# zju-pi/diff-sampler

Measured on AMD Instinct MI355X. Metric: images/sec (whole node) at NFE=10, EDM CIFAR-10, higher is better.
Workload: dtype fp32; 1 GPU; EDM CIFAR-10 32x32 SongUNet (55.7M params), DPM-Solver++(2M) logSNR NFE=10, batch 256/GPU; launch=eager

## Files before the change

### diff_sampler_amd/csrc/conv3x3_wino.hip

```cpp
#include <type_traits>

#include "igemm_common.h"

namespace igemm {
namespace {

typedef float f32x2 __attribute__((ext_vector_type(2)));

constexpr int WV_NO_NORM = 2, WV_NO_HALO = 4, WV_NO_DMA = 8, WV_NO_EPI = 16;
constexpr int WINO_K = 8;
constexpr int WINO_POS = 2 * 64 * 4;
constexpr int WINO_IMG = 16 * WINO_POS;
constexpr int WINO_NSH = 4;
constexpr int WINO_EPI_LD = 36;

#define DS_WINO_WAIT_VM0() do { __builtin_amdgcn_s_waitcnt(0x0F70); asm volatile("" ::: "memory"); } while (0)
#define DS_WINO_WAIT_VM(n) do { __builtin_amdgcn_s_waitcnt(0x0F70 | (n)); asm volatile("" ::: "memory"); } while (0)

#define DS_WINO_I(n) std::integral_constant<int, (n)>{}
#define DS_WINO_EACH4(F) F(0) F(1) F(2) F(3)
#define DS_WINO_EACH8(F) F(0) F(1) F(2) F(3) F(4) F(5) F(6) F(7)
#define DS_WINO_EACH12(F) F(0) F(1) F(2) F(3) F(4) F(5) F(6) F(7) F(8) F(9) F(10) F(11)
#define DS_WINO_EACH16(F, b) F((b) + 0) F((b) + 1) F((b) + 2) F((b) + 3) F((b) + 4) F((b) + 5) F((b) + 6) F((b) + 7)                \
                             F((b) + 8) F((b) + 9) F((b) + 10) F((b) + 11) F((b) + 12) F((b) + 13) F((b) + 14) F((b) + 15)

template <int NT, int NSH, int NSL, int NORM>
struct WinoHalo {
    struct Regs {
        f32x4 h[NSH];
        f32x4 mu = {0.f, 0.f, 0.f, 0.f}, ga = {1.f, 1.f, 1.f, 1.f}, be = {0.f, 0.f, 0.f, 0.f};
    };
    const int c0, Ctot;
    const int buf;
    unsigned off0[NSH], off1[NSH];
    int lds[NSH];
    const float *a0i, *a1i;
    const float* cpi;
    unsigned c_lane;
    float t[4 * NSH], u[4 * NSH];
    const float* h_src = nullptr;
    unsigned h_sel = 0;

    __device__ __forceinline__ WinoHalo(const KParams& p, float* Hs, int tid, int img0, int r0)
        : c0(p.c0), Ctot(p.c0 + p.c1), buf(p.NP * WINO_K + 4) {
        const int kh_h = tid & 1, WPH = p.WP >> 1;
#pragma unroll
        for (int j = 0; j < NSH; ++j) {
            const int hp = (tid + j * NT) >> 1;
            const int hr = hp / p.WP, hc = hp - hr * p.WP;
            const int y = r0 + hr - 1, x = hc - 1;
            const bool in = hp < p.NP;
            const bool ok = in && (unsigned)y < (unsigned)p.H && (unsigned)x < (unsigned)p.W;
            const int pix = min(max(y, 0), p.H - 1) * p.W + min(max(x, 0), p.W - 1);
            off0[j] = (unsigned)(pix * p.lda0 + kh_h * 4) * 4u;
            off1[j] = (unsigned)(pix * p.lda1 + kh_h * 4) * 4u;
            const int cell = (((kh_h * 2 + (hc & 1)) * p.HP + hr) * WPH + (hc >> 1)) * 4;
            lds[j] = ok ? cell : p.NP * WINO_K;
            if (in && !ok) {
                const f32x4 z = {0.f, 0.f, 0.f, 0.f};
                *reinterpret_cast<f32x4*>(Hs + cell) = z;
                *reinterpret_cast<f32x4*>(Hs + buf + cell) = z;
            }
        }
        a0i = p.a0 + (size_t)img0 * p.HW * p.lda0;
        a1i = p.a1 + (size_t)img0 * p.HW * p.lda1;
        cpi = p.norm + (size_t)img0 * 3 * Ctot;
        c_lane = (unsigned)(kh_h * 16);
    }
    __device__ __forceinline__ void src(int s) {
        const int c = s * WINO_K;
        const bool first = c < c0;
        h_src = first ? a0i + c : a1i + (c - c0);
        h_sel = (unsigned)__builtin_amdgcn_readfirstlane(first ? -1 : 0);
        asm volatile("" : "+s"(h_sel));
    }
    template <int J>
    __device__ __forceinline__ void load1(Regs& R, std::integral_constant<int, J>) {
        if constexpr (J < NSL) {
            const unsigned off = (off0[J] & h_sel) | (off1[J] & ~h_sel);
            R.h[J] = *reinterpret_cast<const f32x4*>(reinterpret_cast<const char*>(h_src) + off);
        }
    }
    template <int I>
    __device__ __forceinline__ void coef1(Regs& R, int s, std::integral_constant<int, I>) {
        if constexpr (NORM != 0) {
            const char* cs = reinterpret_cast<const char*>(cpi + (size_t)I * Ctot + s * WINO_K);
            asm volatile("" : "+v"(c_lane));
            const f32x4 v = *reinterpret_cast<const f32x4*>(cs + c_lane);
            if constexpr (I == 0) R.mu = v; else if constexpr (I == 1) R.ga = v; else R.be = v;
        }
    }
    __device__ __forceinline__ void loads(Regs& R, int s) {
#define DS_WINO_F(j) load1(R, DS_WINO_I(j));
        DS_WINO_EACH4(DS_WINO_F)
#undef DS_WINO_F
        coef1(R, s, DS_WINO_I(0)); coef1(R, s, DS_WINO_I(1)); coef1(R, s, DS_WINO_I(2));
    }
    template <int C, int ST>
    __device__ __forceinline__ void chain(Regs& R, float* hs) {
        constexpr int j = C >> 2, e = C & 3;
        if constexpr (j < NSL) {
            if constexpr (ST == 0 && NORM != 0) {
                t[C] = __builtin_fmaf(R.h[j][e] - R.mu[e], R.ga[e], R.be[e]);
                if constexpr (NORM == 2) u[C] = __expf(-t[C]);
            }
            if constexpr (ST == 1 && NORM == 2) u[C] = __builtin_amdgcn_rcpf(1.0f + u[C]);
            if constexpr (ST == 2) {
                float v = R.h[j][e];
                if constexpr (NORM == 1) v = t[C];
                if constexpr (NORM == 2) v = t[C] * u[C];
                R.h[j][e] = v;
                if constexpr (e == 3) *reinterpret_cast<f32x4*>(hs + lds[j]) = R.h[j];
            }
        }
    }
    __device__ __forceinline__ void store(Regs& R, float* hs) {
#define DS_WINO_F(c) chain<c, 0>(R, hs); chain<c, 1>(R, hs); chain<c, 2>(R, hs);
        DS_WINO_EACH16(DS_WINO_F, 0)
#undef DS_WINO_F
    }
};

template <int NT, int ROWS>
struct WinoSkip {
    static constexpr int STEP = NT / 8, NE = 4 * ROWS / STEP;
    int lds[NE];
    int a_off[4];
    unsigned t0, t1;
    const float* src = nullptr;
    unsigned off = 0;
    int step = 0;

    __device__ __forceinline__ WinoSkip(const KParams& p, int tid, int lane, int row0) {
        const int e_chunk = tid & 7, Wt = p.W >> 1;
#pragma unroll
        for (int j = 0; j < NE; ++j) {
            const int lp = (tid >> 3) + STEP * j;
            const int yl = lp / p.W, x = lp - yl * p.W;
            const int ph = (yl & 1) * 2 + (x & 1), t = (yl >> 1) * Wt + (x >> 1);
            lds[j] = (((ph * 4 + (e_chunk >> 1)) * 2 + (e_chunk & 1)) * ROWS + (t ^ e_chunk)) * 4;
        }
#pragma unroll
        for (int g = 0; g < 4; ++g) a_off[g] = ((lane >> 5) * ROWS + ((row0 + (lane & 31)) ^ (2 * g + (lane >> 5)))) * 4;
        t0 = (unsigned)((tid >> 3) * p.elda0 + e_chunk * 4);
        t1 = (unsigned)((tid >> 3) * p.elda1 + e_chunk * 4);
    }
    __device__ __forceinline__ void sel(const KParams& p, int es, int m0) {
        const int c = es * 32;
        const bool first = c < p.ec0;
        const int ld = first ? p.elda0 : p.elda1;
        src = (first ? p.e0 + c : p.e1 + (c - p.ec0)) + (size_t)m0 * ld;
        step = STEP * ld;
        off = first ? t0 : t1;
    }
    template <int J>
    __device__ __forceinline__ void load1(f32x4* dst, std::integral_constant<int, J>) {
        dst[J] = *reinterpret_cast<const f32x4*>(src + (size_t)(J * step) + off);
    }
};

template <auto KERNEL, int NT, int LDS_MAX>
int wino_launch(KParams& p, int smem, hipStream_t stream) {
    DS_ENSURE_DYN_LDS(KERNEL, LDS_MAX);
    hipLaunchKernelGGL(KERNEL, dim3(grid_1d(p.mtiles, p.ntiles)), dim3(NT), smem, stream, p);
    DS_CHECK_LAUNCH();
    return DS_OK;
}

template <typename F>
int wino_by_norm(const KParams& p, F launch) {
    if (!p.norm) return launch(DS_WINO_I(0));
    return p.norm_act == DS_ACT_SILU ? launch(DS_WINO_I(2)) : launch(DS_WINO_I(1));
}

template <int VAR, int NORM, int NSL>
__global__ void __launch_bounds__(256, 1) conv3x3_wino_kernel(const KParams p) {
    extern __shared__ __attribute__((aligned(16))) float smem[];
    float* Us = smem;
    float* Vs = smem + 2 * WINO_IMG;
    float* Hs = smem + 4 * WINO_IMG;

    const int tid = threadIdx.x, lane = tid & 63;
    const int wave = __builtin_amdgcn_readfirstlane(tid >> 6);
    const int wr = wave >> 1, wc = wave & 1;
    int mt, nt;
    if (!decode_tile(blockIdx.x, p.mtiles, p.ntiles, mt, nt)) return;
    const int m0 = mt * 256, n0 = nt * 64;
    const int img0 = m0 / p.HW;
    const int r0 = (m0 - img0 * p.HW) / p.W;
    const int WPH = p.WP >> 1, Wt = p.W >> 1;
    const int Ctot = p.c0 + p.c1;
    const int nslabs = Ctot / WINO_K;
    constexpr bool kDma = !(VAR & WV_NO_DMA), kHalo = !(VAR & WV_NO_HALO);

    constexpr int kNorm = (VAR & WV_NO_NORM) ? 0 : NORM;
    const int kh_h = tid & 1;
    const int h_buf = p.NP * WINO_K + 4;
    unsigned h_off0[WINO_NSH], h_off1[WINO_NSH];
    int h_lds[WINO_NSH];
#pragma unroll
    for (int j = 0; j < WINO_NSH; ++j) {
        const int hp = (tid + j * 256) >> 1;
        const int hr = hp / p.WP, hc = hp - hr * p.WP;
        const int y = r0 + hr - 1, x = hc - 1;
        const bool in = hp < p.NP;
        const bool ok = in && (unsigned)y < (unsigned)p.H && (unsigned)x < (unsigned)p.W;
        const int pix = min(max(y, 0), p.H - 1) * p.W + min(max(x, 0), p.W - 1);
        h_off0[j] = (unsigned)(pix * p.lda0 + kh_h * 4) * 4u;
        h_off1[j] = (unsigned)(pix * p.lda1 + kh_h * 4) * 4u;
        const int cell = (((kh_h * 2 + (hc & 1)) * p.HP + hr) * WPH + (hc >> 1)) * 4;
        h_lds[j] = ok ? cell : p.NP * WINO_K;
        if (in && !ok) {
            const f32x4 z = {0.f, 0.f, 0.f, 0.f};
            *reinterpret_cast<f32x4*>(Hs + cell) = z;
            *reinterpret_cast<f32x4*>(Hs + h_buf + cell) = z;
        }
    }
    const float* a0i = p.a0 + (size_t)img0 * p.HW * p.lda0;
    const float* a1i = p.a1 + (size_t)img0 * p.HW * p.lda1;
    const float* cpi = p.norm + (size_t)img0 * 3 * Ctot;
    unsigned c_lane = (unsigned)(kh_h * 16);
    struct HaloRegs {
        f32x4 h[WINO_NSH];
        f32x4 mu = {0.f, 0.f, 0.f, 0.f}, ga = {1.f, 1.f, 1.f, 1.f}, be = {0.f, 0.f, 0.f, 0.f};
    };
    HaloRegs hreg;
    float h_t[4 * WINO_NSH], h_u[4 * WINO_NSH];
    const float* h_src = nullptr;
    unsigned h_sel = 0;
    auto halo_src = [&](int s) {
        const int c = s * WINO_K;
        const bool first = c < p.c0;
        h_src = first ? a0i + c : a1i + (c - p.c0);
        h_sel = (unsigned)__builtin_amdgcn_readfirstlane(first ? -1 : 0);
        asm volatile("" : "+s"(h_sel));
    };
    auto halo_load1 = [&](HaloRegs& R, auto J) {
        constexpr int j = decltype(J)::value;
        if constexpr (j >= NSL) return;
        const unsigned off = (h_off0[j] & h_sel) | (h_off1[j] & ~h_sel);
        R.h[j] = *reinterpret_cast<const f32x4*>(reinterpret_cast<const char*>(h_src) + off);
    };
    auto coef_load1 = [&](HaloRegs& R, int s, auto I) {
        constexpr int i = decltype(I)::value;
        if constexpr (NORM != 0) {
            const char* cs = reinterpret_cast<const char*>(cpi + (size_t)i * Ctot + s * WINO_K);
            asm volatile("" : "+v"(c_lane));
            const f32x4 v = *reinterpret_cast<const f32x4*>(cs + c_lane);
            if constexpr (i == 0) R.mu = v; else if constexpr (i == 1) R.ga = v; else R.be = v;
        }
    };
    auto halo_chain = [&](HaloRegs& R, float* hs, auto C, auto ST) {
        constexpr int c = decltype(C)::value, st = decltype(ST)::value, j = c >> 2, e = c & 3;
        if constexpr (j >= NSL) return;
        if constexpr (st == 0 && kNorm != 0) {
            h_t[c] = __builtin_fmaf(R.h[j][e] - R.mu[e], R.ga[e], R.be[e]);
            if constexpr (kNorm == 2) h_u[c] = __expf(-h_t[c]);
        }
        if constexpr (st == 1 && kNorm == 2) h_u[c] = __builtin_amdgcn_rcpf(1.0f + h_u[c]);
        if constexpr (st == 2) {
            float v = R.h[j][e];
            if constexpr (kNorm == 1) v = h_t[c];
            if constexpr (kNorm == 2) v = h_t[c] * h_u[c];
            R.h[j][e] = v;
            if constexpr (e == 3) *reinterpret_cast<f32x4*>(hs + h_lds[j]) = R.h[j];
        }
    };

    const int t_t = (tid >> 1) & 63, cpl = tid & 1, kh_t = tid >> 7;
    const int t_ty = t_t / Wt, t_tx = t_t - t_ty * Wt;
    const int h_rd = ((kh_t * 2 * p.HP + 2 * t_ty) * WPH + t_tx) * 4 + cpl * 2;
    const int h_par = p.HP * WPH * 4;
    const int v_wr = (kh_t * 64 + t_t) * 4 + cpl * 2;
    f32x2 t_d[4][4], t_r[4];
    auto tr_read1 = [&](const float* hs, auto I) {
        constexpr int i = decltype(I)::value >> 2, j = decltype(I)::value & 3;
        t_d[i][j] = *reinterpret_cast<const f32x2*>(hs + h_rd + (j & 1) * h_par + i * WPH * 4 + (j >> 1) * 4);
    };
    auto tr_write1 = [&](float* vs, auto I) {
        constexpr int i = decltype(I)::value >> 2, j = decltype(I)::value & 3;
        if constexpr (j == 0) {
#pragma unroll
            for (int q = 0; q < 4; ++q)
                t_r[q] = i == 0 ? t_d[0][q] - t_d[2][q] : i == 1 ? t_d[1][q] + t_d[2][q] : i == 2 ? t_d[2][q] - t_d[1][q] : t_d[1][q] - t_d[3][q];
        }
        const f32x2 v = j == 0 ? t_r[0] - t_r[2] : j == 1 ? t_r[1] + t_r[2] : j == 2 ? t_r[2] - t_r[1] : t_r[1] - t_r[3];
        *reinterpret_cast<f32x2*>(vs + v_wr + (i * 4 + j) * WINO_POS) = v;
    };

    const float* u_src = p.b + (size_t)nt * nslabs * WINO_IMG;
    unsigned u_lane = (unsigned)tid * 16u;
    auto u_dma1 = [&](const float* src, float* ubuf, auto I) {
        constexpr int i = decltype(I)::value;
        float* dst = ubuf + (i * 256 + wave * 64) * 4;
        typedef const __attribute__((address_space(1))) void* gptr_t;
        typedef __attribute__((address_space(3))) void* lptr_t;
        const char* us = reinterpret_cast<const char*>(src + i * 1024);
        asm volatile("" : "+s"(us));
        asm volatile("" : "+v"(u_lane));
        __builtin_amdgcn_global_load_lds((gptr_t)(us + u_lane), (lptr_t)(dst), 16, 0, 0);
    };

    f32x16 acc[16];
#pragma unroll
    for (int q = 0; q < 16; ++q)
#pragma unroll
        for (int r = 0; r < 16; ++r) acc[q][r] = 0.f;
    const int a_off = ((lane >> 5) * 64 + wr * 32 + (lane & 31)) * 4;
    const int b_off = ((lane >> 5) * 64 + wc * 32 + (lane & 31)) * 4;

#define DS_WINO_LOADS(R, sl)                                                                                                           \
    halo_load1(R, DS_WINO_I(0)); halo_load1(R, DS_WINO_I(1)); halo_load1(R, DS_WINO_I(2)); halo_load1(R, DS_WINO_I(3));                \
    coef_load1(R, sl, DS_WINO_I(0)); coef_load1(R, sl, DS_WINO_I(1)); coef_load1(R, sl, DS_WINO_I(2));

    halo_src(0);
    DS_WINO_LOADS(hreg, 0)
    {
        HaloRegs hreg1;
        const int s1 = min(1, nslabs - 1);
        halo_src(s1);
        DS_WINO_LOADS(hreg1, s1)
        DS_RACE_SKEW(wave);
#define DS_WINO_F(i) u_dma1(u_src, Us, DS_WINO_I(i)); u_dma1(u_src, Us, DS_WINO_I((i) + 4));
        DS_WINO_EACH4(DS_WINO_F)
#undef DS_WINO_F
        DS_RACE_SKEW(wave);
#define DS_WINO_CHAIN1(c) halo_chain(hreg, Hs, DS_WINO_I(c), DS_WINO_I(0)); halo_chain(hreg, Hs, DS_WINO_I(c), DS_WINO_I(1));          \
                          halo_chain(hreg, Hs, DS_WINO_I(c), DS_WINO_I(2));
        DS_WINO_EACH16(DS_WINO_CHAIN1, 0)
#undef DS_WINO_CHAIN1
        DS_RACE_SKEW(wave);
#define DS_WINO_CHAIN1(c) halo_chain(hreg1, Hs + h_buf, DS_WINO_I(c), DS_WINO_I(0)); halo_chain(hreg1, Hs + h_buf, DS_WINO_I(c), DS_WINO_I(1)); \
                          halo_chain(hreg1, Hs + h_buf, DS_WINO_I(c), DS_WINO_I(2));
        DS_WINO_EACH16(DS_WINO_CHAIN1, 0)
#undef DS_WINO_CHAIN1
    }
    {
        const int s2 = min(2, nslabs - 1);
        halo_src(s2);
        DS_WINO_LOADS(hreg, s2)
    }
    __syncthreads();
#define DS_WINO_F(i) tr_read1(Hs, DS_WINO_I(i));
    DS_WINO_EACH16(DS_WINO_F, 0)
#undef DS_WINO_F
    DS_RACE_SKEW(wave);
#define DS_WINO_F(i) tr_write1(Vs, DS_WINO_I(i));
    DS_WINO_EACH16(DS_WINO_F, 0)
#undef DS_WINO_F
    DS_WINO_WAIT_VM0();
    __syncthreads();

    f32x4 fa[2][4], fb[2][4];
    int s = 0;
    do {
        const int par = s & 1;
        const float* ub = Us + par * WINO_IMG;
        const float* vb = Vs + par * WINO_IMG;
        float* ubn = Us + (par ^ 1) * WINO_IMG;
        float* vbn = Vs + (par ^ 1) * WINO_IMG;
        float* hb = Hs + par * h_buf;
        const float* hbn = Hs + (par ^ 1) * h_buf;
        const int s1 = min(s + 1, nslabs - 1), s3 = min(s + 3, nslabs - 1);
        const float* un = u_src + (size_t)s1 * WINO_IMG;
// ... 221 lines not shown
    const int wave = __builtin_amdgcn_readfirstlane(tid >> 6);
    int mt, nt;
    if (!decode_tile(blockIdx.x, p.mtiles, p.ntiles, mt, nt)) return;
    const int m0 = mt * 128, n0 = nt * 128;
    const int img0 = m0 / p.HW;
    const int r0 = (m0 - img0 * p.HW) / p.W;
    const int WPH = p.WP >> 1, Wt = p.W >> 1;
    const int Ctot = p.c0 + p.c1;
    const int nslabs = Ctot / WINO_K;

    using Halo = WinoHalo<256, WN_NSH, NSL, NORM>;
    Halo halo(p, Hs, tid, img0, r0);
    const int h_buf = halo.buf;
    typename Halo::Regs hreg;
    auto halo_load1 = [&](typename Halo::Regs& R, auto J) { halo.load1(R, J); };
    auto coef_load1 = [&](typename Halo::Regs& R, int sl, auto I) { halo.coef1(R, sl, I); };

    const int t_t = (tid >> 1) & 31, cpl = tid & 1, kh_t = wave & 1, half = wave >> 1;
    const int t_ty = t_t / Wt, t_tx = t_t - t_ty * Wt;
    const int h_rd = ((kh_t * 2 * p.HP + 2 * t_ty + half) * WPH + t_tx) * 4 + cpl * 2;
    const int h_par = p.HP * WPH * 4;
    const int v_wr = (kh_t * 32 + t_t) * 4 + cpl * 2 + half * 8 * WN_POS;
    f32x2 t_e[3][4];
    auto tr_read1 = [&](const float* hs, auto I) {
        constexpr int i = decltype(I)::value >> 2, j = decltype(I)::value & 3;
        t_e[i][j] = *reinterpret_cast<const f32x2*>(hs + h_rd + (j & 1) * h_par + i * WPH * 4 + (j >> 1) * 4);
    };
    auto tr_write = [&](float* vs) {
        f32x2 ra[4], rb[4];
        if (half == 0) {
#pragma unroll
            for (int q = 0; q < 4; ++q) { ra[q] = t_e[0][q] - t_e[2][q]; rb[q] = t_e[1][q] + t_e[2][q]; }
        } else {
#pragma unroll
            for (int q = 0; q < 4; ++q) { ra[q] = t_e[1][q] - t_e[0][q]; rb[q] = t_e[0][q] - t_e[2][q]; }
        }
#pragma unroll
        for (int i = 0; i < 2; ++i) {
            const f32x2* t_r = i == 0 ? ra : rb;
#pragma unroll
            for (int j = 0; j < 4; ++j) {
                const f32x2 v = j == 0 ? t_r[0] - t_r[2] : j == 1 ? t_r[1] + t_r[2] : j == 2 ? t_r[2] - t_r[1] : t_r[1] - t_r[3];
                *reinterpret_cast<f32x2*>(vs + v_wr + (i * 4 + j) * WN_POS) = v;
            }
        }
    };

    const float* u_src = p.b + (size_t)(2 * nt + (wave >> 1)) * nslabs * WINO_IMG;
    unsigned b_lane = (unsigned)(((lane >> 5) * 64 + (wave & 1) * 32 + (lane & 31)) * 16);
    f32x4 fa[2][4], fb[2][4];
    typedef const __attribute__((address_space(1))) f32x4* gf4_t;
    auto b_load1 = [&](const float* src, auto G, auto I) {
        constexpr int g = decltype(G)::value, i = decltype(I)::value;
        const char* us = reinterpret_cast<const char*>(src + (g * 4 + i) * WINO_POS);
        asm volatile("" : "+s"(us));
        asm volatile("" : "+v"(b_lane));
        fb[g & 1][i] = *(gf4_t)(us + b_lane);
    };

    f32x16 acc[16];
#pragma unroll
    for (int q = 0; q < 16; ++q)
#pragma unroll
        for (int r = 0; r < 16; ++r) acc[q][r] = 0.f;
    const int a_off = ((lane >> 5) * 32 + (lane & 31)) * 4;

    halo.src(0);
    halo.loads(hreg, 0);
    {
        typename Halo::Regs hreg1;
        const int s1 = min(1, nslabs - 1);
        halo.src(s1);
        halo.loads(hreg1, s1);
#define DS_WINO_F(i) b_load1(u_src, DS_WINO_I(0), DS_WINO_I(i));
        DS_WINO_EACH4(DS_WINO_F)
#undef DS_WINO_F
        DS_RACE_SKEW(wave);
        halo.store(hreg, Hs);
        DS_RACE_SKEW(wave);
        halo.store(hreg1, Hs + h_buf);
    }
    {
        const int s2 = min(2, nslabs - 1);
        halo.src(s2);
        halo.loads(hreg, s2);
    }
    __syncthreads();
#define DS_WINO_TR1(i) tr_read1(Hs, DS_WINO_I(i));
    DS_WINO_EACH12(DS_WINO_TR1)
#undef DS_WINO_TR1
    DS_RACE_SKEW(wave);
    tr_write(Vs);
    DS_WINO_WAIT_VM0();
    __syncthreads();

    int s = 0;
    do {
        const int par = s & 1;
        const float* vb = Vs + par * WN_IMG;
        float* vbn = Vs + (par ^ 1) * WN_IMG;
        float* hb = Hs + par * h_buf;
        const float* hbn = Hs + (par ^ 1) * h_buf;
        const int s1 = min(s + 1, nslabs - 1), s3 = min(s + 3, nslabs - 1);
        const float* uc = u_src + (size_t)s * WINO_IMG;
        const float* un = u_src + (size_t)s1 * WINO_IMG;
        auto a_read = [&](auto G, auto I) {
            constexpr int g = decltype(G)::value, i = decltype(I)::value;
            fa[g & 1][i] = *reinterpret_cast<const f32x4*>(vb + (g * 4 + i) * WN_POS + a_off);
        };
#define DS_WINO_TR1(i) tr_read1(hbn, DS_WINO_I(i));
        DS_WINO_EACH12(DS_WINO_TR1)
#undef DS_WINO_TR1
        DS_RACE_SKEW(wave);
        halo.store(hreg, hb);
        halo.src(s3);
        DS_RACE_SKEW(wave);
        tr_write(vbn);
        auto fill = [&](auto K) {
            constexpr int k = decltype(K)::value, g = k >> 4, q = k & 15;
            if constexpr (q < 4) {
                if constexpr (g < 3) b_load1(uc, DS_WINO_I(g + 1), DS_WINO_I(q));
                else b_load1(un, DS_WINO_I(0), DS_WINO_I(q));
            } else if constexpr (k < 7) {
                halo_load1(hreg, DS_WINO_I(k - 4));
            } else if constexpr (k < 10) {
                coef_load1(hreg, s3, DS_WINO_I(k - 7));
            } else if constexpr (q >= 10 && q < 14 && g < 3) {
                a_read(DS_WINO_I(g + 1), DS_WINO_I(q - 10));
            }
        };
#define DS_WINO_STEP(k)                                                                                                                \
        acc[((k) >> 4) * 4 + ((k) & 3)] = __builtin_amdgcn_mfma_f32_32x32x2f32(fa[((k) >> 4) & 1][(k) & 3][((k) >> 2) & 3],            \
                                                                               fb[((k) >> 4) & 1][(k) & 3][((k) >> 2) & 3],            \
                                                                               acc[((k) >> 4) * 4 + ((k) & 3)], 0, 0, 0);              \
        fill(DS_WINO_I(k));                                                                                                            \
        __builtin_amdgcn_sched_barrier(0);
#define DS_WINO_F(i) a_read(DS_WINO_I(0), DS_WINO_I(i));
        DS_WINO_EACH4(DS_WINO_F)
#undef DS_WINO_F
        __builtin_amdgcn_sched_barrier(0);
        DS_WINO_EACH16(DS_WINO_STEP, 0)
        DS_WINO_EACH16(DS_WINO_STEP, 16)
        DS_WINO_EACH16(DS_WINO_STEP, 32)
        DS_WINO_EACH16(DS_WINO_STEP, 48)
#undef DS_WINO_STEP
        __syncthreads();
    } while (++s < nslabs);

    f32x16 Y[4];
#pragma unroll
    for (int a = 0; a < 2; ++a) {
        f32x16 t[4];
#pragma unroll
        for (int j = 0; j < 4; ++j) t[j] = a == 0 ? acc[j] + acc[4 + j] + acc[8 + j] : acc[4 + j] - acc[8 + j] - acc[12 + j];
        Y[a * 2 + 0] = t[0] + t[1] + t[2];
        Y[a * 2 + 1] = t[1] - t[2] - t[3];
    }

    const int nextra = (p.ec0 + p.ec1) / 32;
    if (nextra > 0) {
        const float* wsk = p.b + (size_t)(p.N / 64) * nslabs * WINO_IMG + (size_t)(2 * nt + (wave >> 1)) * nextra * 2048;
        WinoSkip<256, 32> skip(p, tid, lane, 0);
        auto e_load1 = [&](f32x4* dst, auto J) { skip.load1(dst, J); };
        f32x4 ga[2][4], gb[2];
        auto w_load1 = [&](int es, auto G) {
            constexpr int g = decltype(G)::value;
            const char* ws = reinterpret_cast<const char*>(wsk + (size_t)es * 2048 + g * WINO_POS);
            asm volatile("" : "+s"(ws));
            asm volatile("" : "+v"(b_lane));
            gb[g & 1] = *(gf4_t)(ws + b_lane);
        };

        f32x4 ereg[4];
        {
            f32x4 ereg0[4];
            w_load1(0, DS_WINO_I(0));
            skip.sel(p, 0, m0);
#define DS_WINO_F(j) e_load1(ereg0, DS_WINO_I(j));
            DS_WINO_EACH4(DS_WINO_F)
#undef DS_WINO_F
            skip.sel(p, min(1, nextra - 1), m0);
#define DS_WINO_F(j) e_load1(ereg, DS_WINO_I(j));
            DS_WINO_EACH4(DS_WINO_F)
#undef DS_WINO_F
            DS_RACE_SKEW(wave);
#pragma unroll
            for (int j = 0; j < 4; ++j) *reinterpret_cast<f32x4*>(Vs + skip.lds[j]) = ereg0[j];
        }
        __syncthreads();

        int es = 0;
        do {
            const float* vb = smem + (es & 1) * WN_IMG;
            float* vn = smem + ((es + 1) & 1) * WN_IMG;
            const int es1 = min(es + 1, nextra - 1);
            skip.sel(p, min(es + 2, nextra - 1), m0);
            auto a_read = [&](auto G, auto I) {
                constexpr int g = decltype(G)::value, i = decltype(I)::value;
                ga[g & 1][i] = *reinterpret_cast<const f32x4*>(vb + (i * 4 + g) * WN_POS + skip.a_off[g]);
            };
            auto fill = [&](auto K) {
                constexpr int k = decltype(K)::value, g = k >> 4, q = k & 15;
                if constexpr (q == 0) {
                    if constexpr (g < 3) w_load1(es, DS_WINO_I(g + 1));
                    else w_load1(es1, DS_WINO_I(0));
                } else if constexpr (q < 5) {
                    if constexpr (g < 3) a_read(DS_WINO_I(g + 1), DS_WINO_I(q - 1));
                } else if constexpr (k < 9) {
                    if constexpr (k == 5) DS_RACE_SKEW(wave);
                    *reinterpret_cast<f32x4*>(vn + skip.lds[k - 5]) = ereg[k - 5];
                } else if constexpr (k < 13) {
                    e_load1(ereg, DS_WINO_I(k - 9));
                }
            };
#define DS_WINO_STEP(k)                                                                                                                \
            Y[(k) & 3] = __builtin_amdgcn_mfma_f32_32x32x2f32(ga[((k) >> 4) & 1][(k) & 3][((k) >> 2) & 3], gb[((k) >> 4) & 1][((k) >> 2) & 3], \
                                                              Y[(k) & 3], 0, 0, 0);                                                    \
            fill(DS_WINO_I(k));                                                                                                        \
            __builtin_amdgcn_sched_barrier(0);
#define DS_WINO_F(i) a_read(DS_WINO_I(0), DS_WINO_I(i));
            DS_WINO_EACH4(DS_WINO_F)
#undef DS_WINO_F
            __builtin_amdgcn_sched_barrier(0);
            DS_WINO_EACH16(DS_WINO_STEP, 0)
            DS_WINO_EACH16(DS_WINO_STEP, 16)
            DS_WINO_EACH16(DS_WINO_STEP, 32)
            DS_WINO_EACH16(DS_WINO_STEP, 48)
#undef DS_WINO_STEP
            __syncthreads();
        } while (++es < nextra);
    }

    float* stage = smem + wave * 32 * WINO_EPI_LD;
    const int c4 = (lane & 7) * 4;
    const int col = n0 + wave * 32 + c4;
    f32x4 cb = {0.f, 0.f, 0.f, 0.f}, cvu = {0.f, 0.f, 0.f, 0.f};
    if (p.colbias) cb = *reinterpret_cast<const f32x4*>(p.colbias + col);
    if (p.cbias) cvu = *reinterpret_cast<const f32x4*>(p.cbias + (size_t)(p.cbias_bcast ? 0 : img0) * p.cbias_ld + col);
    const float acc_scale = __builtin_bit_cast(float, __builtin_amdgcn_readfirstlane(__builtin_bit_cast(int, p.acc_scale)));
    const float scale = __builtin_bit_cast(float, __builtin_amdgcn_readfirstlane(__builtin_bit_cast(int, p.scale)));
    int e_row[4];
#pragma unroll
    for (int pass = 0; pass < 4; ++pass) {
        const int tl = pass * 8 + (lane >> 3);
        const int ty = tl / Wt, tx = tl - ty * Wt;
        e_row[pass] = m0 + 2 * ty * p.W + 2 * tx;
    }
#pragma unroll
    for (int a = 0; a < 2; ++a) {
        f32x4 st_s = {0.f, 0.f, 0.f, 0.f}, st_q = {0.f, 0.f, 0.f, 0.f};
#pragma unroll
        for (int b = 0; b < 2; ++b) {
            const f32x16 y = Y[a * 2 + b];
            f32x4 rv[4];
            if (p.res) {
#pragma unroll
                for (int pass = 0; pass < 4; ++pass)
                    rv[pass] = __builtin_nontemporal_load(reinterpret_cast<const f32x4*>(p.res + (size_t)(e_row[pass] + a * p.W + b) * p.res_ld + col));
            }
#pragma unroll
            for (int r = 0; r < 16; ++r) stage[((r & 3) + 8 * (r >> 2) + 4 * (lane >> 5)) * WINO_EPI_LD + (lane & 31)] = y[r];
#pragma unroll
            for (int pass = 0; pass < 4; ++pass) {
                f32x4 v = *reinterpret_cast<const f32x4*>(stage + (pass * 8 + (lane >> 3)) * WINO_EPI_LD + c4);
                v *= acc_scale;
                v += cb;
                if (p.cbias) v += cvu;
                if (p.res) v += rv[pass];
                v *= scale;
                if (p.act == DS_ACT_SILU) {
#pragma unroll
                    for (int q = 0; q < 4; ++q) v[q] = ds_silu(v[q]);
                }
                __builtin_nontemporal_store(v, reinterpret_cast<f32x4*>(p.out + (size_t)(e_row[pass] + a * p.W + b) * p.ldo + col));
                st_s += v; st_q += v * v;
            }
        }
        if (p.stats) {
#pragma unroll
            for (int q = 0; q < 4; ++q) {
                st_s[q] += __shfl_xor(st_s[q], 8); st_s[q] += __shfl_xor(st_s[q], 16); st_s[q] += __shfl_xor(st_s[q], 32);
                st_q[q] += __shfl_xor(st_q[q], 8); st_q[q] += __shfl_xor(st_q[q], 16); st_q[q] += __shfl_xor(st_q[q], 32);
            }
            if (lane < 8) {
                float* sp = p.stats + (size_t)((m0 >> 6) + a) * 2 * p.N + col;
                *reinterpret_cast<f32x4*>(sp) = st_s;
                *reinterpret_cast<f32x4*>(sp + p.N) = st_q;
            }
        }
    }
}

int launch_wino_n128(KParams& p, hipStream_t stream) {
    const int smem = (2 * WN_IMG + 2 * (p.NP * WINO_K + 4)) * (int)sizeof(float);
    return wino_by_norm(p, [&](auto NORM) {
        constexpr int norm = decltype(NORM)::value;
        return p.NP * 2 <= 2 * 256 ? wino_launch<wino_n128_kernel<norm, 2>, 256, 64 * 1024>(p, smem, stream)
                                   : wino_launch<wino_n128_kernel<norm, 3>, 256, 64 * 1024>(p, smem, stream);
    });
}

constexpr int W8_NSH = 1;
constexpr int W8_XCH = 4 * 16 * 64;

template <int NORM>
__global__ void __launch_bounds__(512, 1) wino_w8_kernel(const KParams p) {
    extern __shared__ __attribute__((aligned(16))) float smem[];
    float* Vs = smem;
    float* Hs = smem + 2 * WN_IMG;

    const int tid = threadIdx.x, lane = tid & 63;
    const int wave = __builtin_amdgcn_readfirstlane(tid >> 6);
    const int cg = wave & 3, ph = wave >> 2;
    int mt, nt;
    if (!decode_tile(blockIdx.x, p.mtiles, p.ntiles, mt, nt)) return;
    const int m0 = mt * 128, n0 = nt * 128;
    const int img0 = m0 / p.HW;
    const int r0 = (m0 - img0 * p.HW) / p.W;
    const int WPH = p.WP >> 1, Wt = p.W >> 1;
    const int Ctot = p.c0 + p.c1;
    const int nslabs = Ctot / WINO_K;

    using Halo = WinoHalo<512, W8_NSH, W8_NSH, NORM>;
    Halo halo(p, Hs, tid, img0, r0);
    const int h_buf = halo.buf;
    typename Halo::Regs hreg;
    auto halo_load1 = [&](typename Halo::Regs& R, auto J) { halo.load1(R, J); };
    auto coef_load1 = [&](typename Halo::Regs& R, int sl, auto I) { halo.coef1(R, sl, I); };

    const int t_t = (tid >> 1) & 31, cpl = tid & 1, kh_t = wave & 1, t_row = wave >> 1;
    const int t_ty = t_t / Wt, t_tx = t_t - t_ty * Wt;
    const int h_rd0 = ((kh_t * 2 * p.HP + 2 * t_ty + (t_row == 0 ? 0 : 1)) * WPH + t_tx) * 4 + cpl * 2;
    const int h_rd1 = ((kh_t * 2 * p.HP + 2 * t_ty + (t_row == 3 ? 3 : 2)) * WPH + t_tx) * 4 + cpl * 2;
    const int h_par = p.HP * WPH * 4;
    const int v_wr = (kh_t * 32 + t_t) * 4 + cpl * 2 + t_row * 4 * WN_POS;
    f32x2 t_e[2][4];
    auto tr_read1 = [&](const float* hs, auto I) {
        constexpr int i = decltype(I)::value >> 2, j = decltype(I)::value & 3;
        t_e[i][j] = *reinterpret_cast<const f32x2*>(hs + (i == 0 ? h_rd0 : h_rd1) + (j & 1) * h_par + (j >> 1) * 4);
    };
    auto tr_write = [&](float* vs) {
        f32x2 t_r[4];
        if (t_row == 1) {
#pragma unroll
            for (int q = 0; q < 4; ++q) t_r[q] = t_e[0][q] + t_e[1][q];
        } else if (t_row == 2) {
#pragma unroll
            for (int q = 0; q < 4; ++q) t_r[q] = t_e[1][q] - t_e[0][q];
        } else {
#pragma unroll
            for (int q = 0; q < 4; ++q) t_r[q] = t_e[0][q] - t_e[1][q];
        }
#pragma unroll
        for (int j = 0; j < 4; ++j) {
            const f32x2 v = j == 0 ? t_r[0] - t_r[2] : j == 1 ? t_r[1] + t_r[2] : j == 2 ? t_r[2] - t_r[1] : t_r[1] - t_r[3];
            *reinterpret_cast<f32x2*>(vs + v_wr + j * WN_POS) = v;
        }
    };

    const float* u_src = p.b + (size_t)(2 * nt + (cg >> 1)) * nslabs * WINO_IMG + ph * 8 * WINO_POS;
    unsigned b_lane = (unsigned)(((lane >> 5) * 64 + (cg & 1) * 32 + (lane & 31)) * 16);
    f32x4 fa[2][4], fb[2][4];
    typedef const __attribute__((address_space(1))) f32x4* gf4_t;
    auto b_load1 = [&](const float* src, auto G, auto I) {
        constexpr int g = decltype(G)::value, i = decltype(I)::value;
        const char* us = reinterpret_cast<const char*>(src + (g * 4 + i) * WINO_POS);
        asm volatile("" : "+s"(us));
        asm volatile("" : "+v"(b_lane));
        fb[g & 1][i] = *(gf4_t)(us + b_lane);
    };

    f32x16 acc[8];
#pragma unroll
    for (int q = 0; q < 8; ++q)
#pragma unroll
        for (int r = 0; r < 16; ++r) acc[q][r] = 0.f;
    const int a_off = ((lane >> 5) * 32 + (lane & 31)) * 4 + ph * 8 * WN_POS;

    halo.src(0);
    halo.loads(hreg, 0);
    {
        typename Halo::Regs hreg1;
        const int s1 = min(1, nslabs - 1);
        halo.src(s1);
        halo.loads(hreg1, s1);
#define DS_WINO_F(i) b_load1(u_src, DS_WINO_I(0), DS_WINO_I(i));
        DS_WINO_EACH4(DS_WINO_F)
#undef DS_WINO_F
        DS_RACE_SKEW(wave);
        halo.store(hreg, Hs);
        DS_RACE_SKEW(wave);
        halo.store(hreg1, Hs + h_buf);
    }
    {
        const int s2 = min(2, nslabs - 1);
        halo.src(s2);
        halo.loads(hreg, s2);
    }
    __syncthreads();
#define DS_WINO_TR1(i) tr_read1(Hs, DS_WINO_I(i));
    DS_WINO_EACH8(DS_WINO_TR1)
#undef DS_WINO_TR1
    DS_RACE_SKEW(wave);
    tr_write(Vs);
    DS_WINO_WAIT_VM0();
    __syncthreads();

    int s = 0;
    do {
        const int par = s & 1;
        const float* vb = Vs + par * WN_IMG;
        float* vbn = Vs + (par ^ 1) * WN_IMG;
        float* hb = Hs + par * h_buf;
        const float* hbn = Hs + (par ^ 1) * h_buf;
        const int s1 = min(s + 1, nslabs - 1), s3 = min(s + 3, nslabs - 1);
        const float* uc = u_src + (size_t)s * WINO_IMG;
        const float* un = u_src + (size_t)s1 * WINO_IMG;
        auto a_read = [&](auto G, auto I) {
            constexpr int g = decltype(G)::value, i = decltype(I)::value;
            fa[g & 1][i] = *reinterpret_cast<const f32x4*>(vb + (g * 4 + i) * WN_POS + a_off);
        };
#define DS_WINO_TR1(i) tr_read1(hbn, DS_WINO_I(i));
        DS_WINO_EACH8(DS_WINO_TR1)
#undef DS_WINO_TR1
        DS_RACE_SKEW(wave);
        halo.store(hreg, hb);
        halo.src(s3);
        DS_RACE_SKEW(wave);
        tr_write(vbn);
        auto fill = [&](auto K) {
            constexpr int k = decltype(K)::value, g = k >> 4, q = k & 15;
            if constexpr (q < 4) {
                if constexpr (g == 0) b_load1(uc, DS_WINO_I(1), DS_WINO_I(q));
                else b_load1(un, DS_WINO_I(0), DS_WINO_I(q));
            } else if constexpr (k == 4) {
                halo_load1(hreg, DS_WINO_I(0));
            } else if constexpr (k < 8) {
                coef_load1(hreg, s3, DS_WINO_I(k - 5));
            } else if constexpr (k >= 10 && k < 14) {
                a_read(DS_WINO_I(1), DS_WINO_I(k - 10));
            }
        };
#define DS_WINO_STEP(k)                                                                                                                \
        acc[((k) >> 4) * 4 + ((k) & 3)] = __builtin_amdgcn_mfma_f32_32x32x2f32(fa[((k) >> 4) & 1][(k) & 3][((k) >> 2) & 3],            \
                                                                               fb[((k) >> 4) & 1][(k) & 3][((k) >> 2) & 3],            \
                                                                               acc[((k) >> 4) * 4 + ((k) & 3)], 0, 0, 0);              \
        fill(DS_WINO_I(k));                                                                                                            \
        __builtin_amdgcn_sched_barrier(0);
#define DS_WINO_F(i) a_read(DS_WINO_I(0), DS_WINO_I(i));
        DS_WINO_EACH4(DS_WINO_F)
#undef DS_WINO_F
        __builtin_amdgcn_sched_barrier(0);
        DS_WINO_EACH16(DS_WINO_STEP, 0)
        DS_WINO_EACH16(DS_WINO_STEP, 16)
#undef DS_WINO_STEP
        __syncthreads();
    } while (++s < nslabs);

    f32x16 Y[2];
    {
        float* xw = smem + wave * W8_XCH + lane * 4;
        const float* xr = smem + (wave ^ 4) * W8_XCH + lane * 4;
        DS_RACE_SKEW(wave);
#pragma unroll
        for (int q = 0; q < 4; ++q) {
            const f32x16 m = ph == 0 ? acc[4 + q] : acc[q];
#pragma unroll
            for (int r4 = 0; r4 < 4; ++r4) {
                const f32x4 v = {m[4 * r4], m[4 * r4 + 1], m[4 * r4 + 2], m[4 * r4 + 3]};
                *reinterpret_cast<f32x4*>(xw + (q * 4 + r4) * 256) = v;
            }
        }
        __syncthreads();
        f32x16 t[4];
#pragma unroll
        for (int j = 0; j < 4; ++j) {
            f32x16 o;
#pragma unroll
            for (int r4 = 0; r4 < 4; ++r4) {
                const f32x4 v = *reinterpret_cast<const f32x4*>(xr + (j * 4 + r4) * 256);
                o[4 * r4] = v[0]; o[4 * r4 + 1] = v[1]; o[4 * r4 + 2] = v[2]; o[4 * r4 + 3] = v[3];
            }
            if (ph == 0) t[j] = acc[j] + acc[4 + j] + o;
            else t[j] = o - acc[j] - acc[4 + j];
        }
        Y[0] = t[0] + t[1] + t[2];
        Y[1] = t[1] - t[2] - t[3];
    }

    const int nextra = (p.ec0 + p.ec1) / 32;
    if (nextra > 0) {
        __syncthreads();
        const float* wsk = p.b + (size_t)(p.N / 64) * nslabs * WINO_IMG + (size_t)(2 * nt + (cg >> 1)) * nextra * 2048;
        WinoSkip<512, 32> skip(p, tid, lane, 0);
        auto e_load1 = [&](f32x4* dst, auto J) { skip.load1(dst, J); };
        f32x4 ga[2][2], gb[4];
        auto w_load1 = [&](int es, auto G) {
            constexpr int g = decltype(G)::value;
            const char* ws = reinterpret_cast<const char*>(wsk + (size_t)es * 2048 + g * WINO_POS);
            asm volatile("" : "+s"(ws));
            asm volatile("" : "+v"(b_lane));
            gb[g] = *(gf4_t)(ws + b_lane);
        };

        f32x4 ereg[2];
        {
            f32x4 ereg0[2];
            w_load1(0, DS_WINO_I(0)); w_load1(0, DS_WINO_I(1)); w_load1(0, DS_WINO_I(2)); w_load1(0, DS_WINO_I(3));
            skip.sel(p, 0, m0);
            e_load1(ereg0, DS_WINO_I(0)); e_load1(ereg0, DS_WINO_I(1));
            skip.sel(p, min(1, nextra - 1), m0);
            e_load1(ereg, DS_WINO_I(0)); e_load1(ereg, DS_WINO_I(1));
            DS_RACE_SKEW(wave);
#pragma unroll
            for (int j = 0; j < 2; ++j) *reinterpret_cast<f32x4*>(Vs + skip.lds[j]) = ereg0[j];
        }
        __syncthreads();

        int es = 0;
        do {
            const float* vb = smem + (es & 1) * WN_IMG + ph * 8 * WN_POS;
            float* vn = smem + ((es + 1) & 1) * WN_IMG;
            const int es1 = min(es + 1, nextra - 1);
            skip.sel(p, min(es + 2, nextra - 1), m0);
            auto a_read = [&](auto G, auto I) {
                constexpr int g = decltype(G)::value, i = decltype(I)::value;
                ga[g & 1][i] = *reinterpret_cast<const f32x4*>(vb + (i * 4 + g) * WN_POS + skip.a_off[g]);
            };
            auto fill = [&](auto K) {
                constexpr int k = decltype(K)::value, g = k >> 3, q = k & 7;
                if constexpr (q == 0) {
                    if constexpr (g >= 1) w_load1(es1, DS_WINO_I(g - 1));
                } else if constexpr (q < 3) {
                    if constexpr (g < 3) a_read(DS_WINO_I(g + 1), DS_WINO_I(q - 1));
                } else if constexpr (k < 5) {
                    if constexpr (k == 3) DS_RACE_SKEW(wave);
                    *reinterpret_cast<f32x4*>(vn + skip.lds[k - 3]) = ereg[k - 3];
                } else if constexpr (k < 7) {
                    e_load1(ereg, DS_WINO_I(k - 5));
                } else if constexpr (k == 31) {
                    w_load1(es1, DS_WINO_I(3));
                }
            };
#define DS_WINO_STEP(k)                                                                                                                \
            Y[(k) & 1] = __builtin_amdgcn_mfma_f32_32x32x2f32(ga[((k) >> 3) & 1][(k) & 1][((k) >> 1) & 3], gb[(k) >> 3][((k) >> 1) & 3], \
                                                              Y[(k) & 1], 0, 0, 0);                                                    \
            fill(DS_WINO_I(k));                                                                                                        \
            __builtin_amdgcn_sched_barrier(0);
            a_read(DS_WINO_I(0), DS_WINO_I(0)); a_read(DS_WINO_I(0), DS_WINO_I(1));
            __builtin_amdgcn_sched_barrier(0);
            DS_WINO_EACH16(DS_WINO_STEP, 0)
            DS_WINO_EACH16(DS_WINO_STEP, 16)
#undef DS_WINO_STEP
            __syncthreads();
        } while (++es < nextra);
    }

    float* stage = smem + (wave ^ 4) * W8_XCH;
    const int c4 = (lane & 7) * 4;
    const int col = n0 + cg * 32 + c4;
    f32x4 cb = {0.f, 0.f, 0.f, 0.f}, cvu = {0.f, 0.f, 0.f, 0.f};
    if (p.colbias) cb = *reinterpret_cast<const f32x4*>(p.colbias + col);
    if (p.cbias) cvu = *reinterpret_cast<const f32x4*>(p.cbias + (size_t)(p.cbias_bcast ? 0 : img0) * p.cbias_ld + col);
    const float acc_scale = __builtin_bit_cast(float, __builtin_amdgcn_readfirstlane(__builtin_bit_cast(int, p.acc_scale)));
    const float scale = __builtin_bit_cast(float, __builtin_amdgcn_readfirstlane(__builtin_bit_cast(int, p.scale)));
    int e_row[4];
#pragma unroll
    for (int pass = 0; pass < 4; ++pass) {
        const int tl = pass * 8 + (lane >> 3);
        const int ty = tl / Wt, tx = tl - ty * Wt;
        e_row[pass] = m0 + (2 * ty + ph) * p.W + 2 * tx;
    }
    f32x4 st_s = {0.f, 0.f, 0.f, 0.f}, st_q = {0.f, 0.f, 0.f, 0.f};
#pragma unroll
    for (int b = 0; b < 2; ++b) {
        const f32x16 y = Y[b];
        f32x4 rv[4];
        if (p.res) {
#pragma unroll
            for (int pass = 0; pass < 4; ++pass)
                rv[pass] = __builtin_nontemporal_load(reinterpret_cast<const f32x4*>(p.res + (size_t)(e_row[pass] + b) * p.res_ld + col));
        }
#pragma unroll
        for (int r = 0; r < 16; ++r) stage[((r & 3) + 8 * (r >> 2) + 4 * (lane >> 5)) * WINO_EPI_LD + (lane & 31)] = y[r];
#pragma unroll
        for (int pass = 0; pass < 4; ++pass) {
            f32x4 v = *reinterpret_cast<const f32x4*>(stage + (pass * 8 + (lane >> 3)) * WINO_EPI_LD + c4);
            v *= acc_scale;
            v += cb;
            if (p.cbias) v += cvu;
            if (p.res) v += rv[pass];
            v *= scale;
            if (p.act == DS_ACT_SILU) {
#pragma unroll
                for (int q = 0; q < 4; ++q) v[q] = ds_silu(v[q]);
            }
            __builtin_nontemporal_store(v, reinterpret_cast<f32x4*>(p.out + (size_t)(e_row[pass] + b) * p.ldo + col));
            st_s += v; st_q += v * v;
        }
    }
    if (p.stats) {
#pragma unroll
        for (int q = 0; q < 4; ++q) {
            st_s[q] += __shfl_xor(st_s[q], 8); st_s[q] += __shfl_xor(st_s[q], 16); st_s[q] += __shfl_xor(st_s[q], 32);
            st_q[q] += __shfl_xor(st_q[q], 8); st_q[q] += __shfl_xor(st_q[q], 16); st_q[q] += __shfl_xor(st_q[q], 32);
        }
        if (lane < 8) {
            float* sp = p.stats + (size_t)((m0 >> 6) + ph) * 2 * p.N + col;
            *reinterpret_cast<f32x4*>(sp) = st_s;
            *reinterpret_cast<f32x4*>(sp + p.N) = st_q;
        }
    }
}

int launch_wino_w8(KParams& p, hipStream_t stream) {
    const int kloop = (2 * WN_IMG + 2 * (p.NP * WINO_K + 4)) * (int)sizeof(float), xch = 8 * W8_XCH * (int)sizeof(float);
    return wino_by_norm(p, [&](auto NORM) {
        return wino_launch<wino_w8_kernel<decltype(NORM)::value>, 512, 160 * 1024>(p, kloop > xch ? kloop : xch, stream);
    });
}

template <int VAR>
int launch_wino(KParams& p, hipStream_t stream) {
    const int smem = (4 * WINO_IMG + 2 * (p.NP * WINO_K + 4)) * (int)sizeof(float);
    return wino_by_norm(p, [&](auto NORM) {
        constexpr int norm = decltype(NORM)::value;
        return p.NP * 2 <= 3 * 256 ? wino_launch<conv3x3_wino_kernel<VAR, norm, 3>, 256, 160 * 1024>(p, smem, stream)
                                   : wino_launch<conv3x3_wino_kernel<VAR, norm, 4>, 256, 160 * 1024>(p, smem, stream);
    });
}

#undef DS_WINO_EACH16
#undef DS_WINO_EACH12
#undef DS_WINO_EACH8
#undef DS_WINO_EACH4
#undef DS_WINO_I

}

bool conv3x3_wino_applicable(const KParams& p) {
    if (p.taps != 9 || p.stride != 1 || p.splits != 1 || (p.ec0 & 31) || (p.ec1 & 31)) return false;
    if ((p.H & 1) || (p.W & 1) || p.W < 4 || p.W > 64 || p.HW % 256 || 256 % p.W || ((256 / p.W) & 1)) return false;
    if ((p.N & 63) || (p.c0 % WINO_K) || (p.c1 % WINO_K) || !p.vec_ok || p.out_planar || p.out_f16 || p.res_f16 || p.rowbias) return false;
    if (p.act != DS_ACT_NONE && p.act != DS_ACT_SILU) return false;
    const int np = (256 / p.W + 2) * (p.W + 2);
    if (np * 2 > WINO_NSH * 256 || (4 * WINO_IMG + 2 * (np * WINO_K + 4)) * (int)sizeof(float) > 160 * 1024) return false;
    return p.M % 256 == 0;
}

int launch_conv3x3_wino(KParams& p, hipStream_t stream) {
    if (!conv3x3_wino_applicable(p)) return DS_E_SHAPE;
    p.TH = 256 / p.W; p.nimg = 1; p.HP = p.TH + 2; p.WP = p.W + 2; p.NP = p.HP * p.WP;
    p.mtiles = p.M / 256; p.ntiles = p.N / 64; p.n_begin = 0;
#ifdef DS_CONV_ABLATIONS
    if (p.t_variant & 0x10000) {
        switch (p.t_variant & 31) {
            case 2: return launch_wino<2>(p, stream);
            case 4: return launch_wino<4>(p, stream);
            case 8: return launch_wino<8>(p, stream);
            case 16: return launch_wino<16>(p, stream);
            case 28: return launch_wino<28>(p, stream);
            default: break;
        }
    }
#endif
    if (!(p.t_variant & 1024) && p.N % 128 == 0) {
        p.TH = 128 / p.W; p.HP = p.TH + 2; p.NP = p.HP * p.WP;
        p.mtiles = p.M / 128; p.ntiles = p.N / 128;
        const bool w8 = (p.W == 16 || p.W == 32) && !(p.t_variant & 32768);
        return w8 ? launch_wino_w8(p, stream) : launch_wino_n128(p, stream);
    }
    return launch_wino<0>(p, stream);
}

}
```

Measured before the change: 510.5 images/sec.

## Deepen w8 Winograd pipeline with triple V buffers and four halo buffers

The w8 Winograd conv kernel now keeps three transformed-input (V) LDS buffers and four halo buffers. The prologue preloads four slabs of halo and transforms two ahead. In the main loop, the next slab's A-fragment reads and the halo transform reads are spread across the MFMA steps, so LDS latency hides behind compute instead of sitting at the top of each iteration. This costs more LDS per block and more live registers, which may limit occupancy or cause spills. Ablation switches are added to turn each lookahead off.

```diff
diff --git a/diff_sampler_amd/csrc/conv3x3_wino.hip b/diff_sampler_amd/csrc/conv3x3_wino.hip
--- a/diff_sampler_amd/csrc/conv3x3_wino.hip
+++ b/diff_sampler_amd/csrc/conv3x3_wino.hip
@@ -24,7 +24,7 @@
 #define DS_WINO_EACH16(F, b) F((b) + 0) F((b) + 1) F((b) + 2) F((b) + 3) F((b) + 4) F((b) + 5) F((b) + 6) F((b) + 7)                \
                              F((b) + 8) F((b) + 9) F((b) + 10) F((b) + 11) F((b) + 12) F((b) + 13) F((b) + 14) F((b) + 15)
 
-template <int NT, int NSH, int NSL, int NORM>
+template <int NT, int NSH, int NSL, int NORM, int NB = 2>
 struct WinoHalo {
     struct Regs {
         f32x4 h[NSH];
@@ -60,6 +60,8 @@
                 const f32x4 z = {0.f, 0.f, 0.f, 0.f};
                 *reinterpret_cast<f32x4*>(Hs + cell) = z;
                 *reinterpret_cast<f32x4*>(Hs + buf + cell) = z;
+#pragma unroll
+                for (int b = 2; b < NB; ++b) *reinterpret_cast<f32x4*>(Hs + b * buf + cell) = z;
             }
         }
         a0i = p.a0 + (size_t)img0 * p.HW * p.lda0;
@@ -887,12 +889,26 @@
 
 constexpr int W8_NSH = 1;
 constexpr int W8_XCH = 4 * 16 * 64;
-
+constexpr int W8_VR = 3;
+constexpr int W8_HB = 4;
+
+#ifdef DS_CONV_ABLATIONS
+constexpr int WV_NO_AHEAD_A = 32, WV_NO_AHEAD_T = 64;
+#define DS_W8_KERNEL(norm, var) wino_w8_kernel<norm, var>
+template <int NORM, int VAR = 0>
+#else
+#define DS_W8_KERNEL(norm, var) wino_w8_kernel<norm>
 template <int NORM>
+#endif
 __global__ void __launch_bounds__(512, 1) wino_w8_kernel(const KParams p) {
+#ifdef DS_CONV_ABLATIONS
+    constexpr bool kAheadA = !(VAR & WV_NO_AHEAD_A), kAheadT = !(VAR & WV_NO_AHEAD_T);
+#else
+    constexpr bool kAheadA = true, kAheadT = true;
+#endif
     extern __shared__ __attribute__((aligned(16))) float smem[];
     float* Vs = smem;
-    float* Hs = smem + 2 * WN_IMG;
+    float* Hs = smem + W8_VR * WN_IMG;
 
     const int tid = threadIdx.x, lane = tid & 63;
     const int wave = __builtin_amdgcn_readfirstlane(tid >> 6);
@@ -906,7 +922,7 @@
     const int Ctot = p.c0 + p.c1;
     const int nslabs = Ctot / WINO_K;
 
-    using Halo = WinoHalo<512, W8_NSH, W8_NSH, NORM>;
+    using Halo = WinoHalo<512, W8_NSH, W8_NSH, NORM, W8_HB>;
     Halo halo(p, Hs, tid, img0, r0);
     const int h_buf = halo.buf;
     typename Halo::Regs hreg;
@@ -962,57 +978,76 @@
         for (int r = 0; r < 16; ++r) acc[q][r] = 0.f;
     const int a_off = ((lane >> 5) * 32 + (lane & 31)) * 4 + ph * 8 * WN_POS;
 
-    halo.src(0);
-    halo.loads(hreg, 0);
+    const int last = nslabs - 1;
     {
-        typename Halo::Regs hreg1;
-        const int s1 = min(1, nslabs - 1);
-        halo.src(s1);
-        halo.loads(hreg1, s1);
+        typename Halo::Regs h0, h1, h2, h3;
+        halo.src(0);
+        halo.loads(h0, 0);
+        halo.src(min(1, last));
+        halo.loads(h1, min(1, last));
+        halo.src(min(2, last));
+        halo.loads(h2, min(2, last));
+        halo.src(min(3, last));
+        halo.loads(h3, min(3, last));
 #define DS_WINO_F(i) b_load1(u_src, DS_WINO_I(0), DS_WINO_I(i));
         DS_WINO_EACH4(DS_WINO_F)
 #undef DS_WINO_F
         DS_RACE_SKEW(wave);
-        halo.store(hreg, Hs);
-        DS_RACE_SKEW(wave);
-        halo.store(hreg1, Hs + h_buf);
-    }
-    {
-        const int s2 = min(2, nslabs - 1);
-        halo.src(s2);
-        halo.loads(hreg, s2);
-    }
+        halo.store(h0, Hs + 2 * h_buf);
+        DS_RACE_SKEW(wave);
+        halo.store(h1, Hs + 3 * h_buf);
+        DS_RACE_SKEW(wave);
+        halo.store(h2, Hs);
+        DS_RACE_SKEW(wave);
+        halo.store(h3, Hs + h_buf);
+    }
+    halo.src(min(4, last));
+    halo.loads(hreg, min(4, last));
     __syncthreads();
-#define DS_WINO_TR1(i) tr_read1(Hs, DS_WINO_I(i));
+#define DS_WINO_TR1(i) tr_read1(Hs + 2 * h_buf, DS_WINO_I(i));
     DS_WINO_EACH8(DS_WINO_TR1)
 #undef DS_WINO_TR1
     DS_RACE_SKEW(wave);
     tr_write(Vs);
+#define DS_WINO_TR1(i) tr_read1(Hs + 3 * h_buf, DS_WINO_I(i));
+    DS_WINO_EACH8(DS_WINO_TR1)
+#undef DS_WINO_TR1
+    DS_RACE_SKEW(wave);
+    tr_write(Vs + WN_IMG);
+#define DS_WINO_TR1(i) tr_read1(Hs, DS_WINO_I(i));
+    DS_WINO_EACH8(DS_WINO_TR1)
+#undef DS_WINO_TR1
     DS_WINO_WAIT_VM0();
     __syncthreads();
+#define DS_WINO_F(i) fa[0][i] = *reinterpret_cast<const f32x4*>(Vs + (i) * WN_POS + a_off);
+    DS_WINO_EACH4(DS_WINO_F)
+#undef DS_WINO_F
 
     int s = 0;
+    int v0 = 0, v1 = WN_IMG, v2 = 2 * WN_IMG;
     do {
         const int par = s & 1;
-        const float* vb = Vs + par * WN_IMG;
-        float* vbn = Vs + (par ^ 1) * WN_IMG;
+        const float* vb = Vs + v0;
+        const float* vb1 = Vs + v1;
+        float* vb2 = Vs + v2;
         float* hb = Hs + par * h_buf;
         const float* hbn = Hs + (par ^ 1) * h_buf;
-        const int s1 = min(s + 1, nslabs - 1), s3 = min(s + 3, nslabs - 1);
+        const int s1 = min(s + 1, last), s5 = min(s + 5, last);
         const float* uc = u_src + (size_t)s * WINO_IMG;
         const float* un = u_src + (size_t)s1 * WINO_IMG;
-        auto a_read = [&](auto G, auto I) {
+        auto a_read = [&](const float* v, auto G, auto I) {
             constexpr int g = decltype(G)::value, i = decltype(I)::value;
-            fa[g & 1][i] = *reinterpret_cast<const f32x4*>(vb + (g * 4 + i) * WN_POS + a_off);
+            fa[g & 1][i] = *reinterpret_cast<const f32x4*>(v + (g * 4 + i) * WN_POS + a_off);
         };
-#define DS_WINO_TR1(i) tr_read1(hbn, DS_WINO_I(i));
-        DS_WINO_EACH8(DS_WINO_TR1)
-#undef DS_WINO_TR1
+        if constexpr (!kAheadT) {
+#pragma unroll
+            for (int i = 0; i < 8; ++i) asm volatile("" : "+v"(t_e[i >> 2][i & 3]));
+        }
         DS_RACE_SKEW(wave);
         halo.store(hreg, hb);
-        halo.src(s3);
-        DS_RACE_SKEW(wave);
-        tr_write(vbn);
+        halo.src(s5);
+        DS_RACE_SKEW(wave);
+        tr_write(vb2);
         auto fill = [&](auto K) {
             constexpr int k = decltype(K)::value, g = k >> 4, q = k & 15;
             if constexpr (q < 4) {
@@ -1021,9 +1056,18 @@
             } else if constexpr (k == 4) {
                 halo_load1(hreg, DS_WINO_I(0));
             } else if constexpr (k < 8) {
-                coef_load1(hreg, s3, DS_WINO_I(k - 5));
+                coef_load1(hreg, s5, DS_WINO_I(k - 5));
             } else if constexpr (k >= 10 && k < 14) {
-                a_read(DS_WINO_I(1), DS_WINO_I(k - 10));
+                a_read(vb, DS_WINO_I(1), DS_WINO_I(k - 10));
+            } else if constexpr (k >= 24 && k < 28) {
+                if constexpr (kAheadA) a_read(vb1, DS_WINO_I(0), DS_WINO_I(k - 24));
+            } else if constexpr (!kAheadT) {
+            } else if constexpr (k == 8 || k == 9) {
+                tr_read1(hbn, DS_WINO_I(k - 8));
+            } else if constexpr (k == 14 || k == 15) {
+                tr_read1(hbn, DS_WINO_I(k - 12));
+            } else if constexpr (k >= 20 && k < 24) {
+                tr_read1(hbn, DS_WINO_I(k - 16));
             }
         };
 #define DS_WINO_STEP(k)                                                                                                                \
@@ -1032,14 +1076,13 @@
                                                                                acc[((k) >> 4) * 4 + ((k) & 3)], 0, 0, 0);              \
         fill(DS_WINO_I(k));                                                                                                            \
         __builtin_amdgcn_sched_barrier(0);
-#define DS_WINO_F(i) a_read(DS_WINO_I(0), DS_WINO_I(i));
-        DS_WINO_EACH4(DS_WINO_F)
-#undef DS_WINO_F
         __builtin_amdgcn_sched_barrier(0);
         DS_WINO_EACH16(DS_WINO_STEP, 0)
         DS_WINO_EACH16(DS_WINO_STEP, 16)
 #undef DS_WINO_STEP
         __syncthreads();
+        const int v = v0;
+        v0 = v1; v1 = v2; v2 = v;
     } while (++s < nslabs);
 
     f32x16 Y[2];
@@ -1198,12 +1241,14 @@
     }
 }
 
+template <int VAR = 0>
 int launch_wino_w8(KParams& p, hipStream_t stream) {
-    const int kloop = (2 * WN_IMG + 2 * (p.NP * WINO_K + 4)) * (int)sizeof(float), xch = 8 * W8_XCH * (int)sizeof(float);
+    const int kloop = (W8_VR * WN_IMG + W8_HB * (p.NP * WINO_K + 4)) * (int)sizeof(float), xch = 8 * W8_XCH * (int)sizeof(float);
     return wino_by_norm(p, [&](auto NORM) {
-        return wino_launch<wino_w8_kernel<decltype(NORM)::value>, 512, 160 * 1024>(p, kloop > xch ? kloop : xch, stream);
+        return wino_launch<DS_W8_KERNEL(decltype(NORM)::value, VAR), 512, 160 * 1024>(p, kloop > xch ? kloop : xch, stream);
     });
 }
+#undef DS_W8_KERNEL
 
 template <int VAR>
 int launch_wino(KParams& p, hipStream_t stream) {
@@ -1239,6 +1284,14 @@
     p.mtiles = p.M / 256; p.ntiles = p.N / 64; p.n_begin = 0;
 #ifdef DS_CONV_ABLATIONS
     if (p.t_variant & 0x10000) {
+        const int w8v = p.t_variant & (WV_NO_AHEAD_A | WV_NO_AHEAD_T);
+        if (w8v && p.N % 128 == 0 && (p.W == 16 || p.W == 32)) {
+            p.TH = 128 / p.W; p.HP = p.TH + 2; p.NP = p.HP * p.WP;
+            p.mtiles = p.M / 128; p.ntiles = p.N / 128;
+            return w8v == WV_NO_AHEAD_A   ? launch_wino_w8<WV_NO_AHEAD_A>(p, stream)
+                   : w8v == WV_NO_AHEAD_T ? launch_wino_w8<WV_NO_AHEAD_T>(p, stream)
+                                          : launch_wino_w8<WV_NO_AHEAD_A | WV_NO_AHEAD_T>(p, stream);
+        }
         switch (p.t_variant & 31) {
             case 2: return launch_wino<2>(p, stream);
             case 4: return launch_wino<4>(p, stream);
```

After: 513.6 images/sec (median of 6 runs). No clear change (+0.6%).
